# aapo-kossi/gym-eldorado

Measured on AMD Instinct MI355X. Metric: env-steps/sec at n_envs=65536, 4 players; bit-exact vs C++ ref, higher is better.
Workload: dtype u8; 1 GPU; C5: 65,536 envs in total over the ranks, 4 players, HARD, n_pieces=3, max_steps=100000, on-device masked sampler over selected_action_masks + step, persistent rollout kernel, every step's AoS outputs stored in HBM; n_envs_total=65536, n_envs_per_gpu=65536, seed=12345, parallelism=env-sharded x1 by index (runner.h:33-38 block split), no collectives

## Files before the change

gym-eldorado_amd/build_ext.py:

```python
from __future__ import annotations

import os
import subprocess
import sys
import sysconfig

PKG = os.path.dirname(os.path.abspath(__file__))
ROOT = os.path.dirname(PKG)
CSRC = os.path.join(PKG, "csrc")
OUT = os.path.join(PKG, "city_of_gold")
INCLUDE = os.path.join(ROOT, "include")
HIPCC = os.environ.get("HIPCC", "/opt/rocm/bin/hipcc")
ARCH = os.environ.get("COG_OFFLOAD_ARCH", "gfx950")

LIB = os.path.join(OUT, "libcog_hip.so")
LIB_FENCE = os.path.join(OUT, "libcog_hip_fence.so")
EXT = os.path.join(OUT, "_city_of_gold" + sysconfig.get_config_var("EXT_SUFFIX"))

ENGINE_SRCS = [os.path.join(CSRC, f) for f in ("cog_engine.hip", "cog_abi.cpp", "cog_policy.hip")]
ENGINE_DEPS = ENGINE_SRCS + [os.path.join(CSRC, f) for f in ("cog_engine.h", "cog_policy.h", "cog_tables.h", "cog_rng.h")] + [
    os.path.join(INCLUDE, f) for f in ("cog.h", "cog_types.h")]
EXT_SRCS = [os.path.join(CSRC, "pybind_module.cpp")]


def _stale(target, deps):
    if not os.path.exists(target):
        return True
    t = os.path.getmtime(target)
    return any(os.path.getmtime(d) > t for d in deps)


def _run(cmd, cwd=None):
    print("+", " ".join(cmd), flush=True)
    subprocess.run(cmd, check=True, cwd=cwd)


OBJ = os.path.join(PKG, "build")
HEADERS = [os.path.join(CSRC, f) for f in ("cog_engine.h", "cog_policy.h", "cog_tables.h", "cog_rng.h")] + [
    os.path.join(INCLUDE, f) for f in ("cog.h", "cog_types.h")]


def _compile_cmd(src, obj, defs=()):
    return [HIPCC, f"--offload-arch={ARCH}", "-O3", "-std=c++17", "-fPIC", "-c",
            "-ffp-contract=off", "-mllvm", "-amdgpu-sched-strategy=max-ilp", "-falign-loops=64", "-Wall",
            *defs, f"-I{INCLUDE}", f"-I{CSRC}", src, "-o", obj]


def build_engine(force=False, fence=True):
    os.makedirs(OBJ, exist_ok=True)
    jobs, objs = [], []
    for src in ENGINE_SRCS:
        obj = os.path.join(OBJ, os.path.basename(src) + ".o")
        objs.append(obj)
# ... 50 lines not shown
```

gym-eldorado_amd/csrc/cog_abi.cpp:

```cpp
#include <hip/hip_runtime.h>

#include <algorithm>
#include <atomic>
#include <chrono>
#include <cstdlib>
#include <cstring>
#include <mutex>
#include <random>
#include <string>
#include <vector>

#include "../../include/cog.h"
#include "cog_engine.h"
#include "cog_policy.h"

namespace {

thread_local std::string g_err;

int fail(int code, const std::string &msg) {
  g_err = msg;
  return code;
}

// ... 197 lines not shown
  size_t first = 0, n = 0;
  hipStream_t stream = nullptr;
  hipEvent_t ev = nullptr;
  cog::DevState s{};
  uint8_t *outs = nullptr;
  uint8_t *h_outs = nullptr;
  uint8_t *d_actions = nullptr;
  bool status_dirty = false;
  bool zc = false;
  uint8_t *h_obs_d = nullptr, *h_outs_d = nullptr, *mir = nullptr;
  bool mir_valid = false;
  bool host_synced = false, pub_done = false;
  Signal done;
  uint32_t park_seq = 0;
  uint64_t lean_clock = ~0ull;
  bool cdeck_ok = false;
};

struct cog_env {
  size_t n = 0;
  uint8_t n_players = 4;
  uint32_t max_steps = 0;
  uint64_t version = 0;
  std::vector<EnvShard> sh;
  uint32_t *h_err = nullptr;
  bool host = false;
  cog_obs_t *h_obs = nullptr;
  cog_action_mask_t *h_sel = nullptr;
  float *h_rew = nullptr;
  uint8_t *h_done = nullptr;
  uint8_t *h_agent = nullptr;
// ... 91 lines not shown

void env_free(cog_env *e) {
  if (!e) return;
  host_env_register(e, false);
  {
    std::lock_guard<std::mutex> lk(g_host_envs_mu);
    for (cog_sampler *q : g_samplers)
      if (q->spec.env == e) {
        q->spec.ok = false;
        q->spec.env = nullptr;
      }
  }
  for (EnvShard &k : e->sh) {
    DeviceGuard g(k.device);
    if (k.stream) (void)hipStreamSynchronize(k.stream);
    void *dev[] = {k.s.obs, k.outs, k.s.priv, k.s.grid, k.s.cgrid, k.s.heads, k.s.cdeck, k.s.cwide, k.s.gen, k.s.dirty, k.d_actions, k.mir,
                   k.s.park, k.s.parkq, k.done.ctr};
    for (void *p : dev)
      if (p) (void)hipFree(p);
    zc_free(k.h_outs);
    if (k.ev) (void)hipEventDestroy(k.ev);
    if (k.stream) (void)hipStreamDestroy(k.stream);
  }
  zc_free(e->h_obs);
  if (e->h_err) (void)hipHostFree(e->h_err);
  if (!single(e)) {
    void *more[] = {e->h_sel, e->h_rew, e->h_done, e->h_agent, e->h_info};
    for (void *p : more) zc_free(p);
  }
  delete e;
}
// ... 167 lines not shown
    DeviceGuard g(k.device);
    HIPCHK(hipMemcpyAsync(e->h_obs + k.first, k.s.obs, k.n * COG_OBS_BYTES, hipMemcpyDeviceToHost, k.stream));
    HIPCHK(hipMemcpyAsync(k.h_outs + kStatusBytes, k.outs + kStatusBytes, OutLayout(k.n).total - kStatusBytes,
                          hipMemcpyDeviceToHost, k.stream));
  }
  int rc = sync_all(e);
  if (rc) return rc;
  for (EnvShard &k : e->sh) k.mir_valid = false;
  gather_small(e);
  return COG_OK;
}

cog::DevState launch_state(const EnvShard &k, bool host_views) {
  cog::DevState s = k.s;
  if (!host_views) s.cap = 0;
  s.cdeck_ok = k.cdeck_ok ? 1u : 0u;
  return s;
}

void sampler_free(cog_sampler *s) {
  if (!s) return;
  sampler_register(s, false);
  if (!s->sh.empty()) {
    DeviceGuard g(s->sh[0].device);
    if (s->spec.d_rng) (void)hipFree(s->spec.d_rng);
    if (s->spec.d_actions) (void)hipFree(s->spec.d_actions);
  }
  zc_free(s->spec.h);
  for (SamplerShard &k : s->sh) {
    DeviceGuard g(k.device);
    if (k.stream) (void)hipStreamSynchronize(k.stream);
// ... 20 lines not shown
int env_shard_init(EnvShard &k, uint32_t default_seed, uint32_t *err_word) {
  DeviceGuard g(k.device);
  HIPCHK(hipStreamCreateWithFlags(&k.stream, hipStreamNonBlocking));
  HIPCHK(hipEventCreateWithFlags(&k.ev, hipEventDisableTiming));
  const size_t n = k.n;
  const OutLayout L(n);
  cog::DevState &s = k.s;
  int rc;
  if ((rc = dmalloc(&s.obs, n * COG_OBS_BYTES)) || (rc = dmalloc(&k.outs, L.alloc)) ||
      (rc = dmalloc(&s.priv, n * sizeof(cog::EnvPriv))) || (rc = dmalloc(&s.grid, n * (size_t)cog::kGridBytes)) ||
      (rc = dmalloc(&s.cgrid, n * (size_t)COG_CELLS)) || (rc = dmalloc(&s.heads, n * 5 * sizeof(uint4))) ||
      (rc = dmalloc(&s.gen, n * sizeof(cog::GenScratch))) || (rc = dmalloc(&s.dirty, n * sizeof(uint32_t))) ||
      (rc = dmalloc(&k.d_actions, n * COG_ACTION_BYTES)) || (rc = dmalloc(&s.park, n * sizeof(uint32_t))) ||
      (rc = dmalloc(&s.parkq, cog::park_list_bytes(n))) ||
      (rc = dmalloc(&k.done.ctr, 256)) || (rc = zc_alloc(&k.h_outs, L.alloc)) ||
      (rc = dmalloc(&s.cdeck, n * 10 * sizeof(uint4))) || (rc = dmalloc(&s.cwide, n * sizeof(uint32_t))))
    return rc;
  std::memset(k.h_outs, 0, L.alloc);
  s.n = n;
  s.first = k.first;
  s.cap = n;
  s.autoreset = 1;
  s.status = reinterpret_cast<uint32_t *>(k.outs);
  s.sel = k.outs + L.sel;
  s.info = k.outs + L.info;
  s.rew = reinterpret_cast<float *>(k.outs + L.rew);
  s.done = k.outs + L.done;
  s.agent = k.outs + L.agent;
  void *d_err = nullptr;
  HIPCHK(hipHostGetDevicePointer(&d_err, err_word, 0));
  s.err = static_cast<uint32_t *>(d_err);
// ... 95 lines not shown
  return COG_OK;
}

static int env_reset_impl(cog_env *e, const cog::ResetParams &p) {
  int rc = prepare_host(e);
  if (rc) return rc;
  env_changed(e);
  if (p.use_params) {
    e->n_players = p.n_players;
    e->max_steps = p.max_steps;
  }
  for (EnvShard &k : e->sh) {
    k.done.queued = false;
    k.host_synced = false;
    k.lean_clock = e->n_players >= 3 && e->max_steps ? 0ull : ~0ull;
    k.cdeck_ok = false;
  }
  for (EnvShard &k : e->sh) {
    DeviceGuard g(k.device);
    if (cog::launch_reset(k.s, p, k.stream) || cog::launch_encode_all(k.s, k.stream))
      return fail(COG_ERR_HIP, std::string("reset launch failed: ") + hipGetErrorString(hipGetLastError()));
    if ((rc = enqueue_status_only(k))) return rc;
  }
  if ((rc = sync_fast(e))) return rc;
  uint32_t flags = 0, errors = 0;
  for (size_t j = 0; j < e->sh.size(); j++) {
    EnvShard &k = e->sh[j];
    const uint32_t *st = reinterpret_cast<const uint32_t *>(k.h_outs);
    flags |= st[0];
    errors += st[1];
    if (st[0] || st[1] || st[2] || e->h_err[64 * j]) {
// ... 25 lines not shown

int cog_env_step_device_stream(cog_env *env, const void *d_actions, size_t n, void *stream) {
  if (!env || !d_actions) return fail(COG_ERR_INVALID, "NULL argument");
  if (n != env->n) return fail(COG_ERR_INVALID, "actions length != num_envs");
  if (!single(env)) return fail(COG_ERR_INVALID, "device actions need a single-shard env (one device pointer)");
  EnvShard &k = env->sh[0];
  DeviceGuard g(k.device);
  int rc = prepare_host(env);
  if (rc) return rc;
  env_changed(env);
  if (stream != COG_NO_STREAM) {
    HIPCHK(hipEventRecord(k.ev, static_cast<hipStream_t>(stream)));
    HIPCHK(hipStreamWaitEvent(k.stream, k.ev, 0));
  }
  k.lean_clock = ~0ull;
  k.cdeck_ok = false;
  if (cog::launch_step(launch_state(k, env->host), static_cast<const uint8_t *>(d_actions), k.stream))
    return fail(COG_ERR_HIP, std::string("step launch failed: ") + hipGetErrorString(hipGetLastError()));
  return finish(env, true);
}

int cog_env_step_device(cog_env *env, const void *d_actions, size_t n) {
  return cog_env_step_device_stream(env, d_actions, n, COG_NO_STREAM);
}

static bool spec_ready(cog_sampler *q) {
  SamplerSpec &sp = q->spec;
  if (sp.h) return true;
  DeviceGuard g(q->sh[0].device);
  if (dmalloc(&sp.d_rng, q->n * sizeof(uint32_t)) || dmalloc(&sp.d_actions, q->n * COG_ACTION_BYTES) ||
      zc_alloc(&sp.h, q->n * 8 + 64)) {
// ... 14 lines not shown
  if (q && (q->exported || q->sh[0].device != env->sh[0].device || std::getenv("COG_NO_SPEC") || !spec_ready(q)))
    q = nullptr;
  if (q) q->spec.ok = false;
  bool spec_launched = false;
  for (EnvShard &k : env->sh) {
    if (!k.n) continue;
    DeviceGuard g(k.device);
    const uint8_t *da = zc_device(actions + k.first, k.n * COG_ACTION_BYTES);
    if (!da || !zc_same_on(k.device, actions + k.first)) {
      HIPCHK(hipMemcpyAsync(k.d_actions, actions + k.first, k.n * COG_ACTION_BYTES, hipMemcpyHostToDevice, k.stream));
      da = k.d_actions;
    }
    uint32_t seq = 0, *ctr = nullptr;
    k.pub_done = false;
    k.lean_clock = ~0ull;
    k.cdeck_ok = false;
    if (env->host && k.zc && k.mir_valid && k.host_synced && cog::step_pub_ok(k.n) &&
        (ctr = signal_arm(k.done, seq))) {
      cog::DevState ps = launch_state(k, true);
      ps.pub_obs = k.h_obs_d;
      ps.pub_outs = k.h_outs_d;
      ps.pub_mir = k.mir;
      cog::SampleSpec sp{nullptr, nullptr, nullptr, nullptr, nullptr};
      if (q) {
        uint8_t *h = const_cast<uint8_t *>(zc_device(q->spec.h, n * 8 + 64));
        if (h) {
          *reinterpret_cast<volatile uint32_t *>(q->spec.h + n * 8) = 0u;
          sp = cog::SampleSpec{q->sh[0].d_rng, q->spec.d_rng, q->spec.d_actions, h, reinterpret_cast<uint32_t *>(h + n * 8)};
          spec_launched = true;
        }
      }
// ... 118 lines not shown
  }
  int rc = sync_all(env);
  if (rc) return rc;
  uint32_t acc = 0;
  for (uint32_t f : tmp) acc |= f;
  if (flags_or) *flags_or = acc;
  if (per_env) std::memcpy(per_env, tmp.data(), tmp.size() * sizeof(uint32_t));
  return COG_OK;
}

int cog_env_clear_hazards(cog_env *env) {
  if (!env) return fail(COG_ERR_INVALID, "env is NULL");
  for (EnvShard &k : env->sh) {
    if (!k.n) continue;
    DeviceGuard g(k.device);
    HIPCHK(hipMemset2DAsync(reinterpret_cast<uint8_t *>(k.s.priv) + offsetof(cog::EnvPriv, flags), sizeof(cog::EnvPriv),
                            0, sizeof(uint32_t), k.n, k.stream));
  }
  return sync_all(env);
}

int cog_env_time_encode(cog_env *env, int iters, int variant, double *ms_per_launch) {
  if (!env || iters < 1 || !ms_per_launch) return fail(COG_ERR_INVALID, "bad argument");
  EnvShard &k = env->sh[0];
  DeviceGuard g(k.device);
  hipEvent_t e0, e1;
  HIPCHK(hipEventCreate(&e0));
  HIPCHK(hipEventCreate(&e1));
  if (cog::launch_encode_all(k.s, k.stream, variant))
    return fail(COG_ERR_HIP, "encode launch failed");
// ... 86 lines not shown
  return COG_OK;
}

int cog_env_invalidate_device(cog_env *env, void *stream) {
  if (!env) return fail(COG_ERR_INVALID, "env is NULL");
  int rc = prepare_host(env);
  if (rc) return rc;
  env_changed(env);
  for (EnvShard &k : env->sh) {
    DeviceGuard g(k.device);
    if (stream != COG_NO_STREAM) {
      HIPCHK(hipEventRecord(k.ev, static_cast<hipStream_t>(stream)));
      HIPCHK(hipStreamWaitEvent(k.stream, k.ev, 0));
    }
    k.lean_clock = ~0ull;
    k.cdeck_ok = false;
    if (cog::launch_resync(k.s, k.stream))
      return fail(COG_ERR_HIP, std::string("resync launch failed: ") + hipGetErrorString(hipGetLastError()));
  }
  return finish(env, true);
}

int cog_env_set_autoreset(cog_env *env, int on) {
  if (!env) return fail(COG_ERR_INVALID, "env is NULL");
  int rc = sync_all(env);
  if (rc) return rc;
  env_changed(env);
  for (EnvShard &k : env->sh) {
    k.s.autoreset = on ? 1u : 0u;
    k.lean_clock = ~0ull;
    k.cdeck_ok = false;
  }
  return COG_OK;
}

int cog_sampler_create_multi(size_t n_envs, uint64_t seed, const int *devices, int n_devices, cog_sampler **out) {
  return cog_sampler_create_at(n_envs, seed, 0, devices, n_devices, out);
}

int cog_sampler_create_at(size_t n_envs, uint64_t seed, uint64_t first_index, const int *devices, int n_devices,
                          cog_sampler **out) {
  if (!out) return fail(COG_ERR_INVALID, "out is NULL");
  *out = nullptr;
  int rc = check_devices(devices, n_devices);
  if (rc) return rc;
  cog_sampler *s = new cog_sampler();
// ... 343 lines not shown
}

static int runner_launch_fused(cog_runner *r, int steps) {
  const int src = (r->flags & COG_RUNNER_STORED_MASKS) ? cog::MASK_STORED : cog::MASK_SELECTED;
  env_changed(r->env);
  r->smp->version++;
  const bool host = runner_host(r);
  int rc;
  if (host && (rc = prepare_host(r->env))) return rc;
  for (size_t j = 0; j < r->env->sh.size(); j++) {
    EnvShard &k = r->env->sh[j];
    SamplerShard &q = r->smp->sh[j];
    DeviceGuard g(k.device);
    if (host && steps == 1 && !r->timing && k.zc && k.mir_valid && k.host_synced && cog::step_pub_ok(k.n) && q.n) {
      k.lean_clock = ~0ull;
      k.cdeck_ok = false;
      uint8_t *h_act = const_cast<uint8_t *>(zc_device(r->smp->h_actions + q.first, q.n * COG_ACTION_BYTES));
      uint32_t seq = 0, *ctr = nullptr;
      if (h_act && zc_same_on(k.device, r->smp->h_actions + q.first) && (ctr = signal_arm(k.done, seq))) {
        cog::DevState ps = launch_state(k, true);
        ps.pub_obs = k.h_obs_d;
        ps.pub_outs = k.h_outs_d;
        ps.pub_mir = k.mir;
        if (cog::launch_sample_step_pub(ps, src, q.d_rng, q.d_actions, h_act, k.stream, ctr, k.done.d, seq))
          return fail(COG_ERR_HIP, std::string("sample_step launch failed: ") + hipGetErrorString(hipGetLastError()));
        signal_armed(k.done);
        k.pub_done = true;
        continue;
      }
    }
    views_pending(k);
    if (r->timing) {
      if ((rc = runner_timing_event(r, j))) return rc;
      HIPCHK(hipEventRecord(r->ev[j][r->ev_used], k.stream));
    }
    const cog::DevState s = launch_state(k, host);
    if (r->chunk > 1) {
      const bool trio = cog::rollout_kind_of(k.n, src, r->env->n_players >= 3) == 3;
      for (int t = 0; t < steps; t += r->chunk) {
        const int kk = std::min(r->chunk, steps - t);
        const bool no_fixup = trio && k.s.autoreset && k.lean_clock != ~0ull &&
                              k.lean_clock + (uint64_t)kk < (uint64_t)r->env->max_steps;
        cog::DevState sc = s;
        sc.cdeck_ok = trio && k.cdeck_ok ? 1u : 0u;
#ifdef COG_NO_CDECK
        sc.cdeck_ok = 0u;
#endif
        if (cog::launch_rollout(sc, src, kk, q.d_rng, q.d_actions, k.stream, r->env->n_players >= 3, &k.park_seq,
                                no_fixup))
          return fail(COG_ERR_HIP, std::string("rollout launch failed: ") + hipGetErrorString(hipGetLastError()));
        k.lean_clock = trio && k.lean_clock != ~0ull ? k.lean_clock + (uint64_t)kk : ~0ull;
        k.cdeck_ok = trio;
      }
    } else {
      k.lean_clock = ~0ull;
      k.cdeck_ok = false;
      for (int t = 0; t < steps; t++)
        if (cog::launch_sample_step(s, src, q.d_rng, q.d_actions, k.stream))
          return fail(COG_ERR_HIP, std::string("sample_step launch failed: ") + hipGetErrorString(hipGetLastError()));
    }
    if (r->timing) HIPCHK(hipEventRecord(r->ev[j][r->ev_used + 1], k.stream));
  }
  if (r->timing) {
    r->ev_used += 2;
    r->timed_launches += (uint64_t)steps;
  }
  return COG_OK;
}

int cog_runner_sample(cog_runner *r) {
  if (!r) return fail(COG_ERR_INVALID, "runner is NULL");
// ... 6 lines not shown
int cog_runner_step(cog_runner *r) {
  if (!r) return fail(COG_ERR_INVALID, "runner is NULL");
  env_changed(r->env);
  if (r->pending_sample) {
    r->pending_sample = false;
    return runner_launch_fused(r, 1);
  }
  const bool host = runner_host(r);
  int rc;
  if (host && (rc = prepare_host(r->env))) return rc;
  for (EnvShard &k : r->env->sh) views_pending(k);
  for (size_t j = 0; j < r->env->sh.size(); j++) {
    EnvShard &k = r->env->sh[j];
    DeviceGuard g(k.device);
    k.lean_clock = ~0ull;
    k.cdeck_ok = false;
    if (cog::launch_step(launch_state(k, host), r->smp->sh[j].d_actions, k.stream))
      return fail(COG_ERR_HIP, std::string("step launch failed: ") + hipGetErrorString(hipGetLastError()));
  }
  return COG_OK;
}

int cog_runner_rollout(cog_runner *r, int steps) {
  if (!r || steps < 0) return fail(COG_ERR_INVALID, "bad argument");
  int rc = runner_flush_sample(r);
  if (rc) return rc;
  return steps ? runner_launch_fused(r, steps) : COG_OK;
}

int cog_runner_sync(cog_runner *r) {
  if (!r) return fail(COG_ERR_INVALID, "runner is NULL");
// ... 53 lines not shown
```

gym-eldorado_amd/csrc/cog_engine.h:

```cpp
#pragma once
#include <stddef.h>
#include <stdint.h>

#include "../../include/cog_types.h"

namespace cog {

constexpr int kGridDim = 128;
constexpr int kGridOff = 64;
constexpr int kGridBytes = kGridDim * kGridDim;
#define COG_CELLS 2304
constexpr int kMaxCoord = 62;
constexpr int kMaxPlaced = 96;

constexpr uint32_t F_MAPGEN_FAIL = 0x01u;
constexpr uint32_t F_ERASE_PAST = 0x02u;
constexpr uint32_t F_Q9_OOB = 0x04u;
constexpr uint32_t F_Q24_CLAMP = 0x08u;
constexpr uint32_t F_GRID_OVER = 0x10u;
constexpr uint32_t F_OOB_LOOKUP = 0x20u;
constexpr uint32_t F_SCAN_OVER = 0x40u;
constexpr uint32_t F_B_START_LT4 = 0x80u;
constexpr uint32_t F_BAD_ACTION = 0x100u;
constexpr uint32_t F_SYNC_TIMEOUT = 0x200u;
// ... 34 lines not shown
};
static_assert(sizeof(GenScratch) <= 256, "GenScratch");

struct DevState {
  size_t n;
  uint8_t *obs;
  uint8_t *sel;
  uint8_t *info;
  float *rew;
  uint8_t *done;
  uint8_t *agent;
  EnvPriv *priv;
  uint8_t *grid;
  uint8_t *cgrid;
  uint4 *heads;
  uint4 *cdeck;
  uint32_t *cwide;
  GenScratch *gen;
  uint32_t *status;
  uint32_t *dirty;
  uint32_t *err;
  size_t first;
  size_t cap;
  uint32_t autoreset;
  unsigned long long *stamps;
  uint32_t *park;
  uint32_t *parkq;
  uint32_t park_par;
  uint32_t no_fixup;
  uint32_t trio_jt;
  uint32_t cdeck_ok;
  uint8_t *pub_obs, *pub_outs, *pub_mir;
  int32_t redo_at;
  int32_t redo_env;
};

struct ResetParams {
  uint32_t seed;
  uint8_t n_players, n_pieces, difficulty, use_params;
  uint32_t max_steps;
};

enum MaskSource : int { MASK_SELECTED = 0, MASK_STORED = 1, MASK_EXTERNAL = 2 };

int launch_init(const DevState &s, const uint32_t *seeds_host_unused, uint32_t default_seed,
                void *stream);
// ... 37 lines not shown
```

gym-eldorado_amd/csrc/cog_engine.hip:

```cpp
#include <hip/hip_runtime.h>
#include <algorithm>
#include <cstdlib>
#include <cstring>

#include "cog_engine.h"
#include "cog_tables.h"
#include "cog_rng.h"

#define DEV __device__ __forceinline__

#ifdef COG_STAMPS
DEV unsigned long long stamp_clock() {
  unsigned long long t;
  __builtin_amdgcn_sched_barrier(0);
  asm volatile("s_memtime %0\n\ts_waitcnt lgkmcnt(0)" : "=s"(t) :: "memory");
  __builtin_amdgcn_sched_barrier(0);
  return t;
}
#define STAMP(s, k)                                                                          \
  do {                                                                                       \
    const unsigned long long t_ = stamp_clock();                                             \
    if ((s).stamps && (threadIdx.x & 63) == 0)                                               \
      (s).stamps[((size_t)blockIdx.x * (blockDim.x / 64) + threadIdx.x / 64) * 16 + (k)] = t_; \
  } while (0)
// ... 2006 lines not shown

DEV void load_env(const DevState &s, size_t i, Snap &S) {
  const uint4 *pv4 = reinterpret_cast<const uint4 *>(s.priv + i);
  const uint4 *sh4 = reinterpret_cast<const uint4 *>(s.obs + i * COG_OBS_BYTES + COG_OBS_PHASE);
  S.g0 = pv4[0];
  S.g1 = pv4[1];
  S.g2 = pv4[2];
  S.info_steps = reinterpret_cast<const uint32_t *>(pv4 + 3)[0];
  S.sel = mbits_of(s.heads[5 * i]);
  S.sh[0] = sh4[0];
  S.sh[1] = sh4[1];
  S.sh[2] = sh4[2];
  const uint32_t w[5] = {S.sh[1].x, S.sh[1].y, S.sh[1].z, S.sh[1].w, S.sh[2].x};
  S.avail = shop_avail_of(w, (S.g1.y >> 8) & 0xffu, S.g1.z);
}
DEV uint8_t *deck_ptr(const DevState &s, size_t i, int p) {
  return s.obs + i * COG_OBS_BYTES + COG_OBS_PLAYER0 + COG_OBS_PLAYER_STRIDE * p;
}
DEV void load_players(const DevState &s, size_t i, int ag, int na, Snap &S) {
  const uint4 *pv4 = reinterpret_cast<const uint4 *>(s.priv + i);
  S.pla = pv4[4 + ag];
  S.pln = pv4[4 + na];
  S.ca = reinterpret_cast<const uint2 *>(pv4 + 8)[ag];
  S.cn = reinterpret_cast<const uint2 *>(pv4 + 8)[na];
  S.sta = mbits_of(s.heads[5 * i + 1 + ag]);
  S.stn = mbits_of(s.heads[5 * i + 1 + na]);
  const uint4 *dk = reinterpret_cast<const uint4 *>(deck_ptr(s, i, ag));
#pragma unroll
  for (int k = 0; k < 7; k++) S.dk[k] = dk[k];
}
// ... 382 lines not shown

constexpr uint32_t kParkNone = ~0u, kParkFinish = 1u << 31, kParkRedo = 1u << 30;
constexpr uint32_t kParkStep = kParkRedo - 1u;
DEV DevState wave_view(const DevState &s, size_t base) {
  DevState v = s;
  v.obs += base * COG_OBS_BYTES;
  v.sel += base * COG_MASK_BYTES;
  v.info += base * COG_INFO_BYTES;
  v.rew += base * 4;
  v.done += base;
  v.agent += base;
  v.priv += base;
  v.grid += base * (size_t)kGridBytes;
  v.cgrid += base * COG_CELLS;
  v.heads += 5 * base;
  v.cdeck += 10 * base;
  v.cwide += base;
  v.gen += base;
  v.park += base;
  v.first += base;
  v.n = s.n > base ? s.n - base : 0;
  return v;
}
DEV void park_list_push(const DevState &s_glob, bool parked) {
  if (__builtin_amdgcn_ballot_w64(parked) && (threadIdx.x & 63) == 0) {
    if (s_glob.no_fixup) {
      atomicOr(&s_glob.status[0], F_PARK_NOFIX);
      atomicAdd(&s_glob.status[1], 1u);
      *s_glob.err = 1u;
    }
    const uint32_t j = atomicAdd(&s_glob.parkq[s_glob.park_par], 1u);
// ... 787 lines not shown
  const int ne = (int)min((size_t)epw, s_glob.n - wbase);
  uint32_t *__restrict__ rngs = rngs_glob + wbase;
  bool live = l < ne;
  uint32_t park = kParkNone, srng = 0;
  PH_DECL;
  TL(10);
  RegEnv R;
  uint2 cells[4];
  int te1 = -1, te2 = -1;
  int ag = 0, na = 0;
  MBits selb = {0u, 0u, 0u}, stab = selb, stnb = selb;
  constexpr bool lat = LAT;
  uint4 pp = make_uint4(0u, 0u, 0u, 0u);
  uint32_t n_in_hand = 0u, n_active = 0u, steps_taken = 0u;
  uint32_t own = 0u;
  if (live) {
    Snap S;
    load_env(s, i, S);
    regs_env(R, S);
    const uint4 *pv4 = reinterpret_cast<const uint4 *>(s.priv + i);
#pragma unroll
    for (int p = 0; p < 4; p++) {
      D.pl[p][l] = pv4[4 + p];
      cells[p] = reinterpret_cast<const uint2 *>(pv4 + 8)[p];
      D.heads[p][l] = s.heads[5 * i + 1 + p];
    }
    srng = rngs[i];
    ag = (int)R.agent();
    na = (int)next_player((uint32_t)ag, R.n_players());
    pp = D.pl[ag][l];
    n_in_hand = (pp.y >> 8) & 0xffu;
    n_active = (pp.y >> 16) & 0xffu;
    steps_taken = (pp.z >> 8) & 0xffu;
#pragma unroll
    for (int p = 0; p < 4; p++) own |= (cells[p].x & 0xffu) << (8 * p);
    selb = S.sel;
    stab = mbits_of(D.heads[ag][l]);
    stnb = mbits_of(D.heads[na][l]);
  }
  R.tab = D.tab;
  __builtin_amdgcn_s_waitcnt(0);
// ... 177 lines not shown
      live = false;
    }
    ag = ag1;
    na = na1;
    PH(3);
  }
  TL(12);
  if (live && !lat) D.pl[ag][l] = pack_lean_player(pp, n_in_hand, n_active, steps_taken);
  cnt_store(D, CNT_REC, (uint32_t)steps + 1u);
  uint4 *pw = reinterpret_cast<uint4 *>(s.priv + i);
  if (lat) {
    if (live) {
      reinterpret_cast<uint3 *>(reinterpret_cast<uint32_t *>(pw) + 1)[0] = make_uint3(R.seed, R.max_steps, R.turn_counter);
      s.heads[5 * i] = mbits_u4(selb);
      rngs[i] = srng;
    }
    if (l < ne) s.park[i] = park;
    park_list_push(s_glob, park != kParkNone);
  }
  cnt_wait(D, cc, cc.fin, 3u, s_glob);
  PH(7);
  TL(13);
  const uint32_t fl = D.flg[l];
  if (lat) {
    if (live) pw[1] = make_uint4(R.g1x, R.g1y, R.in_market, R.flags | fl);
    else if (l < ne && fl) reinterpret_cast<uint32_t *>(pw)[7] = R.flags | fl;
  } else {
    if (live) {
      R.flags |= fl;
      trio_store_private(s, i, R, selb);
      rngs[i] = srng;
    } else if (l < ne && fl) {
      reinterpret_cast<uint32_t *>(pw)[7] = R.flags | fl;
    }
    if (l < ne) s.park[i] = park;
    park_list_push(s_glob, park != kParkNone);
  }
  trio_store_players(D, s, ne);
  PH(8);
  TL(14);
  PH_FLUSH(s_glob);
}

template <bool LAT>
DEV void trio_draw_play(TrioLds &D, const DevState &s, int l, bool live, int slot, uint32_t mt, uint32_t w2,
                        uint32_t gx, uint4 &p4, uint2 &h, uint2 &a, uint4 &shb0, uint32_t &infob, bool &te,
                        bool &rec_out, uint32_t &dm, uint32_t &nact) {
  const size_t i = (size_t)l;
  const int ag = (int)((mt >> 2) & 3u);
  const bool valid = live && (mt & kMetaValid);
  const bool rec = valid && (mt & kMetaStepped);
  rec_out = rec;
  te = rec && (int)(mt >> 24) != ag;
// ... 57 lines not shown

template <bool LAT>
DEV uint32_t trio_drawer(TrioLds &D, const DevState &s_glob, int steps, int epw) {
  PH_DECL;
  TL(14);
  const int l = (int)(threadIdx.x & 63);
  const size_t wbase = (size_t)blockIdx.x * epw;
  const DevState s = wave_view(s_glob, wbase);
  const size_t i = (size_t)l;
  const bool live = l < epw && wbase + (size_t)l < s_glob.n;
  uint32_t rng = 0u;
  bool narrow = true;
  constexpr bool lat = LAT;
  uint4 shb0 = make_uint4(0u, 0u, 0u, 0u);
  uint32_t infob = 0u;
  if (live && !s_glob.cdeck_ok) {
#pragma unroll
    for (int p = 0; p < 4; p++) {
      const uint4 *src = reinterpret_cast<const uint4 *>(deck_ptr(s, i, p));
      uint4 dk[7];
      uint2 pile[5];
#pragma unroll
      for (int k = 0; k < 7; k++) dk[k] = src[k];
      narrow = compact_of(dk, pile) && narrow;
#pragma unroll
      for (int q = 0; q < 5; q++) D.img[p][q][l] = pile[q];
    }
  }
  if (live) {
    rng = reinterpret_cast<const uint32_t *>(s.priv + i)[0];
    infob = reinterpret_cast<const uint32_t *>(s.priv + i)[12];
    shb0 = reinterpret_cast<const uint4 *>(s.obs + i * COG_OBS_BYTES + COG_OBS_PHASE)[0];
  }
  if (!s_glob.cdeck_ok) D.wide[l] = narrow ? 0u : 1u;
  uint32_t flags = 0u;
  __builtin_amdgcn_s_waitcnt(0);
  TL(15);
  __syncthreads();
  PH_RESET;
  TrioCnt6 cc;
  for (int r = 0; r < steps; r += 2) {
    const int nrec = r + 1 < steps ? 2 : 1;
    cnt_wait(D, cc, cc.rec, (uint32_t)(r + nrec), s_glob);
    PH(8);
    if (r + nrec >= steps) TL(11);
    const int slot[2] = {r & (kTrioDepth - 1), (r + 1) & (kTrioDepth - 1)};
    uint32_t dm[2] = {0u, 0u}, nact[2] = {0u, 0u};
    int agj[2] = {0, 0};
    bool te[2] = {false, false}, recj[2] = {false, false};
// ... 45 lines not shown
    }
#pragma unroll
    for (int j = 0; j < 2; j++)
      if (j < nrec) {
        uint32_t *w = &D.ring[slot[j]][2][l].w;
        if (lat && recj[j]) *w = (*w & 0xffu) | nact[j] << 8 | dm[j] << 16;
        else reinterpret_cast<uint16_t *>(w)[1] = (uint16_t)dm[j];
      }
    cnt_store(D, CNT_DRAW, (uint32_t)(r + nrec));
    PH(9);
  }
  TL(12);
  if (live) {
    reinterpret_cast<uint32_t *>(s.priv + i)[0] = rng;
    reinterpret_cast<uint32_t *>(s.priv + i)[12] = infob;
  }
  PH_FLUSH(s_glob);
  return flags;
}

template <int PART, bool LAT>
DEV uint32_t trio_storer(TrioLds &D, const DevState &s_glob, int steps, int epw, const uint32_t *__restrict__ rngs_glob,
                         uint8_t *__restrict__ actions_glob) {
  PH_DECL;
  TL(14);
  const int l = (int)(threadIdx.x & 63);
  const size_t wbase = (size_t)blockIdx.x * epw;
  const DevState s = wave_view(s_glob, wbase);
  const size_t i = (size_t)l;
  const bool live = l < epw && wbase + (size_t)l < s_glob.n;
  uint8_t *__restrict__ av = actions_glob + wbase * COG_ACTION_BYTES;
  MBits selb = {0u, 0u, 0u};
  uint2 cells[4];
  uint32_t out = ~0u;
  RegEnv E;
  E.flags = 0u;
  E.avail = 0u;
  uint32_t x = 1u;
  if (live) {
    if (PART == 0) {
      const uint4 *sh4 = reinterpret_cast<const uint4 *>(s.obs + i * COG_OBS_BYTES + COG_OBS_PHASE);
      const uint4 sh1 = sh4[1], sh2 = sh4[2];
      const uint4 *pv4 = reinterpret_cast<const uint4 *>(s.priv + i);
#pragma unroll
      for (int p = 0; p < 4; p++) {
        D.stbA[p][l] = s.heads[5 * i + 1 + p];
        cells[p] = reinterpret_cast<const uint2 *>(pv4 + 8)[p];
      }
      const uint4 g1 = pv4[1];
      const uint32_t w[5] = {sh1.x, sh1.y, sh1.z, sh1.w, sh2.x};
      E.avail = shop_avail_of(w, (g1.y >> 8) & 0xffu, g1.z);
      if (s_glob.cdeck_ok) {
        const uint4 *src = s.cdeck + 10 * i;
        uint4 c[10];
#pragma unroll
        for (int g = 0; g < 10; g++) c[g] = src[g];
#pragma unroll
        for (int g = 0; g < 10; g++) {
          D.img[(2 * g) / 5][(2 * g) % 5][l] = make_uint2(c[g].x, c[g].y);
          D.img[(2 * g + 1) / 5][(2 * g + 1) % 5][l] = make_uint2(c[g].z, c[g].w);
        }
      }
    } else {
      selb = mbits_of(s.heads[5 * i]);
      x = rngs_glob[wbase + (size_t)l];
    }
  }
  if (PART == 0 && s_glob.cdeck_ok) D.wide[l] = live ? s.cwide[i] : 0u;
  if (PART == 1) {
#pragma unroll
    for (int k = 0; k < kTrioLead; k++) {
      const uint4 p = presample(x);
      D.pre[k][l] = pre_pack(p, LAT);
      x = p.z;
    }
  }
  __builtin_amdgcn_s_waitcnt(0);
  TL(15);
  __syncthreads();
  PH_RESET;
  constexpr int LAG = PART == 1 ? kTrioBLag : 0;
  auto deck_rec = [&](int q) {
    const int sl = q & (kTrioDepth - 1);
// ... 74 lines not shown
        D.stbA[na][l] = mbits_u4(bn);
      }
    }
    if (PART == 1) {
      deck_rec(q);
    } else {
      cnt_store(D, CNT_STA, (uint32_t)(q + 1));
    }
    PH(13);
  }
  TL(12);
  if (PART == 0) {
    cnt_wait(D, cc, cc.rec, (uint32_t)steps + 1u, s_glob);
    if (live) {
#pragma unroll
      for (int p = 0; p < 4; p++) D.heads[p][l] = D.stbA[p][l];
      uint4 *dst = s.cdeck + 10 * i;
#pragma unroll
      for (int g = 0; g < 10; g++) {
        const uint2 a = D.img[(2 * g) / 5][(2 * g) % 5][l], b = D.img[(2 * g + 1) / 5][(2 * g + 1) % 5][l];
        dst[g] = make_uint4(a.x, a.y, b.x, b.y);
      }
      s.cwide[i] = D.wide[l];
    }
  }
  PH_FLUSH(s_glob);
  return E.flags;
}

template <int SRC, bool LAT>
__global__ void __launch_bounds__(256) __attribute__((amdgpu_waves_per_eu(4))) k_env_rollout_trio(DevState s, int steps, int epw, uint32_t *__restrict__ rngs,
                                                          uint8_t *__restrict__ actions_out) {
  __shared__ TrioLds D;
  const int role = __builtin_amdgcn_readfirstlane((int)(threadIdx.x >> 6));
  if (threadIdx.x < 64) D.flg[threadIdx.x] = 0u;
  if (threadIdx.x < kTrioCnts) D.cnt[threadIdx.x] = 0u;
// ... 13 lines not shown
  if (l == 0) __hip_atomic_fetch_add(&D.cnt[CNT_FIN], 1u, __ATOMIC_RELEASE, __HIP_MEMORY_SCOPE_WORKGROUP);
}

template <int SRC>
__global__ void __launch_bounds__(64) k_env_fixup(DevState s, int steps, uint32_t *__restrict__ rngs,
                                                  uint8_t *__restrict__ actions_out, int epw) {
  __shared__ LaneLds<64> L;
  const uint32_t cnt = s.parkq[s.park_par];
  if (blockIdx.x >= cnt) return;
  uid_tab_fill(L.tab);
  for (uint32_t w = blockIdx.x; w < cnt; w += gridDim.x) {
    const size_t base = (size_t)s.parkq[2 + w] * (size_t)epw;
    const size_t i0 = base + threadIdx.x;
    const uint32_t park = (int)threadIdx.x < epw && i0 < s.n ? s.park[i0] : kParkNone;
    rollout_pass<SRC, true, 64>(L, s, steps, rngs, actions_out, park, nullptr, base);
    if (park != kParkNone) {
      const int l = (int)threadIdx.x;
      uint4 *pw = reinterpret_cast<uint4 *>(s.priv + i0);
#pragma unroll
      for (int p = 0; p < 4; p++) {
        pw[4 + p] = L.pl[p][l];
        reinterpret_cast<uint2 *>(pw + 8)[p] = L.cells[p][l];
        s.heads[5 * i0 + 1 + p] = L.heads[p][l];
      }
      bool narrow = true;
#pragma unroll
      for (int p = 0; p < 4; p++) {
        const uint4 *src = reinterpret_cast<const uint4 *>(deck_ptr(s, i0, p));
        uint4 dk[7];
        uint2 pile[5];
#pragma unroll
        for (int k = 0; k < 7; k++) dk[k] = src[k];
        narrow = compact_of(dk, pile) && narrow;
        uint2 *dst = reinterpret_cast<uint2 *>(s.cdeck + 10 * i0) + 5 * p;
#pragma unroll
        for (int q = 0; q < 5; q++) dst[q] = pile[q];
      }
      s.cwide[i0] = narrow ? 0u : 1u;
      s.park[i0] = kParkNone;
    }
  }
}

__global__ void __launch_bounds__(256) k_sample(size_t n, const uint8_t *__restrict__ masks,
                                                uint32_t *__restrict__ rngs, uint8_t *__restrict__ actions,
                                                uint8_t *__restrict__ h_actions, GridSignal sig) {
  __shared__ UidEntry tab[kUidTab];
  uid_tab_fill(tab);
  const size_t i = (size_t)blockIdx.x * blockDim.x + threadIdx.x;
  if (i < n) {
    uint32_t rng = rngs[i];
    uint8_t a[5];
// ... 305 lines not shown
    }();
    DevState sd = s;
    sd.redo_at = park_nofix.first >= 0 ? park_nofix.first : redo_at;
    sd.redo_env = park_nofix.first >= 0 ? (int32_t)park_nofix.second : -1;
    sd.park_par = (*park_seq)++ & 1u;
    static const bool always_fixup = getenv("COG_ALWAYS_FIXUP") != nullptr;
    sd.no_fixup = no_fixup && kind == RK_TRIO && (redo_at < 0 || park_nofix.first >= 0) && !always_fixup ? 1u : 0u;
    const int epw = kind == RK_TRIO ? trio_epw(s.n) : 64;
    const unsigned nb = blocks_for(s.n, epw);
    const dim3 g(nb), gf(fixup_grid(nb));
    static const int jt_env = [] {
      const char *e = getenv("COG_TRIO_JT");
      return e && *e ? atoi(e) : -1;
    }();
    sd.trio_jt = jt_env >= 0 ? (uint32_t)(jt_env != 0) : (nb <= cu_shape().cus ? 1u : 0u);
    if (mask_source == MASK_STORED) {
      hipLaunchKernelGGL((k_env_rollout_duo<MASK_STORED>), g, dim3(128), 0, st, sd, steps, d_rng, d_actions);
      hipLaunchKernelGGL((k_env_fixup<MASK_STORED>), gf, dim3(64), 0, st, sd, steps, d_rng, d_actions, epw);
    } else if (kind == RK_TRIO) {
      if (sd.trio_jt)
        hipLaunchKernelGGL((k_env_rollout_trio<MASK_SELECTED, true>), g, dim3(256), trio_pad_lds(nb), st, sd, steps, epw,
                           d_rng, d_actions);
      else
        hipLaunchKernelGGL((k_env_rollout_trio<MASK_SELECTED, false>), g, dim3(256), trio_pad_lds(nb), st, sd, steps, epw,
                           d_rng, d_actions);
      if (!sd.no_fixup)
        hipLaunchKernelGGL((k_env_fixup<MASK_SELECTED>), gf, dim3(64), 0, st, sd, steps, d_rng, d_actions, epw);
    } else {
      hipLaunchKernelGGL((k_env_rollout_duo<MASK_SELECTED>), g, dim3(128), 0, st, sd, steps, d_rng, d_actions);
      hipLaunchKernelGGL((k_env_fixup<MASK_SELECTED>), gf, dim3(64), 0, st, sd, steps, d_rng, d_actions, epw);
// ... 77 lines not shown
```

Measured before the change: 25.89 billion env-steps/s.

## Carry per-env rollout state across launches in a coalesced SoA carry buffer

Replaces the per-env compact deck buffer with a wider carry buffer laid out in 64-env blocks of 28 uint4 planes, so each lane reads and writes one 16-byte granule per plane. The buffer holds decks, private globals, player state, cells, heads and shop words. Later rollout launches reload state from it with coalesced loads instead of scattered AoS reads from priv, heads and obs. The cost is extra stores on every launch to keep the carry current, plus invalidation logic at reset and on every non-trio path; a stale carry would break bit-exactness.

```diff
diff --git a/gym-eldorado_amd/build_ext.py b/gym-eldorado_amd/build_ext.py
--- a/gym-eldorado_amd/build_ext.py
+++ b/gym-eldorado_amd/build_ext.py
@@ -18,7 +18,7 @@
 EXT = os.path.join(OUT, "_city_of_gold" + sysconfig.get_config_var("EXT_SUFFIX"))
 
 ENGINE_SRCS = [os.path.join(CSRC, f) for f in ("cog_engine.hip", "cog_abi.cpp", "cog_policy.hip")]
-ENGINE_DEPS = ENGINE_SRCS + [os.path.join(CSRC, f) for f in ("cog_engine.h", "cog_policy.h", "cog_tables.h", "cog_rng.h")] + [
+ENGINE_DEPS = ENGINE_SRCS + [os.path.join(CSRC, f) for f in ("cog_engine.h", "cog_policy.h", "cog_tables.h", "cog_rng.h", "cog_carry.h")] + [
     os.path.join(INCLUDE, f) for f in ("cog.h", "cog_types.h")]
 EXT_SRCS = [os.path.join(CSRC, "pybind_module.cpp")]
 
@@ -36,7 +36,7 @@
 
 
 OBJ = os.path.join(PKG, "build")
-HEADERS = [os.path.join(CSRC, f) for f in ("cog_engine.h", "cog_policy.h", "cog_tables.h", "cog_rng.h")] + [
+HEADERS = [os.path.join(CSRC, f) for f in ("cog_engine.h", "cog_policy.h", "cog_tables.h", "cog_rng.h", "cog_carry.h")] + [
     os.path.join(INCLUDE, f) for f in ("cog.h", "cog_types.h")]
 
 
diff --git a/gym-eldorado_amd/csrc/cog_abi.cpp b/gym-eldorado_amd/csrc/cog_abi.cpp
--- a/gym-eldorado_amd/csrc/cog_abi.cpp
+++ b/gym-eldorado_amd/csrc/cog_abi.cpp
@@ -235,7 +235,7 @@
   Signal done;
   uint32_t park_seq = 0;
   uint64_t lean_clock = ~0ull;
-  bool cdeck_ok = false;
+  bool carry_ok = false;
 };
 
 struct cog_env {
@@ -357,7 +357,7 @@
   for (EnvShard &k : e->sh) {
     DeviceGuard g(k.device);
     if (k.stream) (void)hipStreamSynchronize(k.stream);
-    void *dev[] = {k.s.obs, k.outs, k.s.priv, k.s.grid, k.s.cgrid, k.s.heads, k.s.cdeck, k.s.cwide, k.s.gen, k.s.dirty, k.d_actions, k.mir,
+    void *dev[] = {k.s.obs, k.outs, k.s.priv, k.s.grid, k.s.cgrid, k.s.heads, k.s.carry, k.s.cwide, k.s.gen, k.s.dirty, k.d_actions, k.mir,
                    k.s.park, k.s.parkq, k.done.ctr};
     for (void *p : dev)
       if (p) (void)hipFree(p);
@@ -555,7 +555,7 @@
 cog::DevState launch_state(const EnvShard &k, bool host_views) {
   cog::DevState s = k.s;
   if (!host_views) s.cap = 0;
-  s.cdeck_ok = k.cdeck_ok ? 1u : 0u;
+  s.carry_ok = k.carry_ok ? 1u : 0u;
   return s;
 }
 
@@ -606,7 +606,7 @@
       (rc = dmalloc(&k.d_actions, n * COG_ACTION_BYTES)) || (rc = dmalloc(&s.park, n * sizeof(uint32_t))) ||
       (rc = dmalloc(&s.parkq, cog::park_list_bytes(n))) ||
       (rc = dmalloc(&k.done.ctr, 256)) || (rc = zc_alloc(&k.h_outs, L.alloc)) ||
-      (rc = dmalloc(&s.cdeck, n * 10 * sizeof(uint4))) || (rc = dmalloc(&s.cwide, n * sizeof(uint32_t))))
+      (rc = dmalloc(&s.carry, cog::carry_granules(n) * sizeof(uint4))) || (rc = dmalloc(&s.cwide, n * sizeof(uint32_t))))
     return rc;
   std::memset(k.h_outs, 0, L.alloc);
   s.n = n;
@@ -732,7 +732,7 @@
     k.done.queued = false;
     k.host_synced = false;
     k.lean_clock = e->n_players >= 3 && e->max_steps ? 0ull : ~0ull;
-    k.cdeck_ok = false;
+    k.carry_ok = false;
   }
   for (EnvShard &k : e->sh) {
     DeviceGuard g(k.device);
@@ -788,7 +788,7 @@
     HIPCHK(hipStreamWaitEvent(k.stream, k.ev, 0));
   }
   k.lean_clock = ~0ull;
-  k.cdeck_ok = false;
+  k.carry_ok = false;
   if (cog::launch_step(launch_state(k, env->host), static_cast<const uint8_t *>(d_actions), k.stream))
     return fail(COG_ERR_HIP, std::string("step launch failed: ") + hipGetErrorString(hipGetLastError()));
   return finish(env, true);
@@ -833,7 +833,7 @@
     uint32_t seq = 0, *ctr = nullptr;
     k.pub_done = false;
     k.lean_clock = ~0ull;
-    k.cdeck_ok = false;
+    k.carry_ok = false;
     if (env->host && k.zc && k.mir_valid && k.host_synced && cog::step_pub_ok(k.n) &&
         (ctr = signal_arm(k.done, seq))) {
       cog::DevState ps = launch_state(k, true);
@@ -982,6 +982,7 @@
   for (EnvShard &k : env->sh) {
     if (!k.n) continue;
     DeviceGuard g(k.device);
+    k.carry_ok = false;
     HIPCHK(hipMemset2DAsync(reinterpret_cast<uint8_t *>(k.s.priv) + offsetof(cog::EnvPriv, flags), sizeof(cog::EnvPriv),
                             0, sizeof(uint32_t), k.n, k.stream));
   }
@@ -1098,7 +1099,7 @@
       HIPCHK(hipStreamWaitEvent(k.stream, k.ev, 0));
     }
     k.lean_clock = ~0ull;
-    k.cdeck_ok = false;
+    k.carry_ok = false;
     if (cog::launch_resync(k.s, k.stream))
       return fail(COG_ERR_HIP, std::string("resync launch failed: ") + hipGetErrorString(hipGetLastError()));
   }
@@ -1113,7 +1114,7 @@
   for (EnvShard &k : env->sh) {
     k.s.autoreset = on ? 1u : 0u;
     k.lean_clock = ~0ull;
-    k.cdeck_ok = false;
+    k.carry_ok = false;
   }
   return COG_OK;
 }
@@ -1487,7 +1488,7 @@
     DeviceGuard g(k.device);
     if (host && steps == 1 && !r->timing && k.zc && k.mir_valid && k.host_synced && cog::step_pub_ok(k.n) && q.n) {
       k.lean_clock = ~0ull;
-      k.cdeck_ok = false;
+      k.carry_ok = false;
       uint8_t *h_act = const_cast<uint8_t *>(zc_device(r->smp->h_actions + q.first, q.n * COG_ACTION_BYTES));
       uint32_t seq = 0, *ctr = nullptr;
       if (h_act && zc_same_on(k.device, r->smp->h_actions + q.first) && (ctr = signal_arm(k.done, seq))) {
@@ -1515,19 +1516,19 @@
         const bool no_fixup = trio && k.s.autoreset && k.lean_clock != ~0ull &&
                               k.lean_clock + (uint64_t)kk < (uint64_t)r->env->max_steps;
         cog::DevState sc = s;
-        sc.cdeck_ok = trio && k.cdeck_ok ? 1u : 0u;
+        sc.carry_ok = trio && k.carry_ok ? 1u : 0u;
 #ifdef COG_NO_CDECK
-        sc.cdeck_ok = 0u;
+        sc.carry_ok = 0u;
 #endif
         if (cog::launch_rollout(sc, src, kk, q.d_rng, q.d_actions, k.stream, r->env->n_players >= 3, &k.park_seq,
                                 no_fixup))
           return fail(COG_ERR_HIP, std::string("rollout launch failed: ") + hipGetErrorString(hipGetLastError()));
         k.lean_clock = trio && k.lean_clock != ~0ull ? k.lean_clock + (uint64_t)kk : ~0ull;
-        k.cdeck_ok = trio;
+        k.carry_ok = trio;
       }
     } else {
       k.lean_clock = ~0ull;
-      k.cdeck_ok = false;
+      k.carry_ok = false;
       for (int t = 0; t < steps; t++)
         if (cog::launch_sample_step(s, src, q.d_rng, q.d_actions, k.stream))
           return fail(COG_ERR_HIP, std::string("sample_step launch failed: ") + hipGetErrorString(hipGetLastError()));
@@ -1564,7 +1565,7 @@
     EnvShard &k = r->env->sh[j];
     DeviceGuard g(k.device);
     k.lean_clock = ~0ull;
-    k.cdeck_ok = false;
+    k.carry_ok = false;
     if (cog::launch_step(launch_state(k, host), r->smp->sh[j].d_actions, k.stream))
       return fail(COG_ERR_HIP, std::string("step launch failed: ") + hipGetErrorString(hipGetLastError()));
   }
diff --git a/gym-eldorado_amd/csrc/cog_carry.h b/gym-eldorado_amd/csrc/cog_carry.h
--- /dev/null
+++ b/gym-eldorado_amd/csrc/cog_carry.h
@@ -0,0 +1,29 @@
+#pragma once
+#include <stddef.h>
+#include <stdint.h>
+
+#ifndef COG_HD
+#define COG_HD __host__ __device__ __forceinline__
+#endif
+
+namespace cog {
+
+enum CarryPlane : int {
+  kCarryDeck = 0,
+  kCarryG0 = 10,
+  kCarryG1 = 11,
+  kCarryG2 = 12,
+  kCarryDraw = 13,
+  kCarryPl = 14,
+  kCarryCells = 18,
+  kCarryHeads = 20,
+  kCarryObs = 25,
+  kCarryPlanes = 28
+};
+constexpr size_t kCarryBlock = 64;
+
+COG_HD size_t carry_granules(size_t n) { return (n + kCarryBlock - 1) / kCarryBlock * (size_t)kCarryPlanes * kCarryBlock; }
+COG_HD size_t carry_base(size_t e) { return e / kCarryBlock * (size_t)kCarryPlanes * kCarryBlock + e % kCarryBlock; }
+COG_HD size_t carry_slot(size_t e, int g) { return carry_base(e) + (size_t)g * kCarryBlock; }
+
+}
diff --git a/gym-eldorado_amd/csrc/cog_engine.h b/gym-eldorado_amd/csrc/cog_engine.h
--- a/gym-eldorado_amd/csrc/cog_engine.h
+++ b/gym-eldorado_amd/csrc/cog_engine.h
@@ -3,6 +3,7 @@
 #include <stdint.h>
 
 #include "../../include/cog_types.h"
+#include "cog_carry.h"
 
 namespace cog {
 
@@ -72,7 +73,7 @@
   uint8_t *grid;
   uint8_t *cgrid;
   uint4 *heads;
-  uint4 *cdeck;
+  uint4 *carry;
   uint32_t *cwide;
   GenScratch *gen;
   uint32_t *status;
@@ -87,7 +88,7 @@
   uint32_t park_par;
   uint32_t no_fixup;
   uint32_t trio_jt;
-  uint32_t cdeck_ok;
+  uint32_t carry_ok;
   uint8_t *pub_obs, *pub_outs, *pub_mir;
   int32_t redo_at;
   int32_t redo_env;
diff --git a/gym-eldorado_amd/csrc/cog_engine.hip b/gym-eldorado_amd/csrc/cog_engine.hip
--- a/gym-eldorado_amd/csrc/cog_engine.hip
+++ b/gym-eldorado_amd/csrc/cog_engine.hip
@@ -2044,6 +2044,18 @@
   const uint32_t w[5] = {S.sh[1].x, S.sh[1].y, S.sh[1].z, S.sh[1].w, S.sh[2].x};
   S.avail = shop_avail_of(w, (S.g1.y >> 8) & 0xffu, S.g1.z);
 }
+DEV void load_env_carry(const uint4 *ci, Snap &S) {
+  S.g0 = ci[64 * kCarryG0];
+  S.g1 = ci[64 * kCarryG1];
+  S.g2 = ci[64 * kCarryG2];
+  S.info_steps = 0u;
+  S.sel = mbits_of(ci[64 * kCarryHeads]);
+  S.sh[0] = ci[64 * kCarryObs];
+  S.sh[1] = ci[64 * (kCarryObs + 1)];
+  S.sh[2] = ci[64 * (kCarryObs + 2)];
+  const uint32_t w[5] = {S.sh[1].x, S.sh[1].y, S.sh[1].z, S.sh[1].w, S.sh[2].x};
+  S.avail = shop_avail_of(w, (S.g1.y >> 8) & 0xffu, S.g1.z);
+}
 DEV uint8_t *deck_ptr(const DevState &s, size_t i, int p) {
   return s.obs + i * COG_OBS_BYTES + COG_OBS_PLAYER0 + COG_OBS_PLAYER_STRIDE * p;
 }
@@ -2456,7 +2468,7 @@
   v.grid += base * (size_t)kGridBytes;
   v.cgrid += base * COG_CELLS;
   v.heads += 5 * base;
-  v.cdeck += 10 * base;
+  v.carry += carry_base(base);
   v.cwide += base;
   v.gen += base;
   v.park += base;
@@ -3274,17 +3286,37 @@
   uint4 pp = make_uint4(0u, 0u, 0u, 0u);
   uint32_t n_in_hand = 0u, n_active = 0u, steps_taken = 0u;
   uint32_t own = 0u;
+  uint4 *const ci = s.carry + l;
   if (live) {
     Snap S;
-    load_env(s, i, S);
+    if (s_glob.carry_ok) {
+      load_env_carry(ci, S);
+      const uint4 c0 = ci[64 * kCarryCells], c1 = ci[64 * (kCarryCells + 1)];
+      cells[0] = make_uint2(c0.x, c0.y);
+      cells[1] = make_uint2(c0.z, c0.w);
+      cells[2] = make_uint2(c1.x, c1.y);
+      cells[3] = make_uint2(c1.z, c1.w);
+#pragma unroll
+      for (int p = 0; p < 4; p++) {
+        D.pl[p][l] = ci[64 * (kCarryPl + p)];
+        D.heads[p][l] = ci[64 * (kCarryHeads + 1 + p)];
+      }
+    } else {
+      load_env(s, i, S);
+      const uint4 *pv4 = reinterpret_cast<const uint4 *>(s.priv + i);
+#pragma unroll
+      for (int p = 0; p < 4; p++) {
+        D.pl[p][l] = pv4[4 + p];
+        cells[p] = reinterpret_cast<const uint2 *>(pv4 + 8)[p];
+        D.heads[p][l] = s.heads[5 * i + 1 + p];
+      }
+      ci[64 * kCarryG2] = S.g2;
+      ci[64 * kCarryCells] = make_uint4(cells[0].x, cells[0].y, cells[1].x, cells[1].y);
+      ci[64 * (kCarryCells + 1)] = make_uint4(cells[2].x, cells[2].y, cells[3].x, cells[3].y);
+      ci[64 * (kCarryObs + 1)] = S.sh[1];
+      ci[64 * (kCarryObs + 2)] = S.sh[2];
+    }
     regs_env(R, S);
-    const uint4 *pv4 = reinterpret_cast<const uint4 *>(s.priv + i);
-#pragma unroll
-    for (int p = 0; p < 4; p++) {
-      D.pl[p][l] = pv4[4 + p];
-      cells[p] = reinterpret_cast<const uint2 *>(pv4 + 8)[p];
-      D.heads[p][l] = s.heads[5 * i + 1 + p];
-    }
     srng = rngs[i];
     ag = (int)R.agent();
     na = (int)next_player((uint32_t)ag, R.n_players());
@@ -3492,6 +3524,8 @@
       reinterpret_cast<uint3 *>(reinterpret_cast<uint32_t *>(pw) + 1)[0] = make_uint3(R.seed, R.max_steps, R.turn_counter);
       s.heads[5 * i] = mbits_u4(selb);
       rngs[i] = srng;
+      ci[64 * kCarryG0] = make_uint4(0u, R.seed, R.max_steps, R.turn_counter);
+      ci[64 * kCarryHeads] = mbits_u4(selb);
     }
     if (l < ne) s.park[i] = park;
     park_list_push(s_glob, park != kParkNone);
@@ -3501,13 +3535,18 @@
   TL(13);
   const uint32_t fl = D.flg[l];
   if (lat) {
-    if (live) pw[1] = make_uint4(R.g1x, R.g1y, R.in_market, R.flags | fl);
-    else if (l < ne && fl) reinterpret_cast<uint32_t *>(pw)[7] = R.flags | fl;
+    if (live) {
+      pw[1] = make_uint4(R.g1x, R.g1y, R.in_market, R.flags | fl);
+      ci[64 * kCarryG1] = make_uint4(R.g1x, R.g1y, R.in_market, R.flags | fl);
+    } else if (l < ne && fl) reinterpret_cast<uint32_t *>(pw)[7] = R.flags | fl;
   } else {
     if (live) {
       R.flags |= fl;
       trio_store_private(s, i, R, selb);
       rngs[i] = srng;
+      ci[64 * kCarryG0] = make_uint4(0u, R.seed, R.max_steps, R.turn_counter);
+      ci[64 * kCarryG1] = make_uint4(R.g1x, R.g1y, R.in_market, R.flags);
+      ci[64 * kCarryHeads] = mbits_u4(selb);
     } else if (l < ne && fl) {
       reinterpret_cast<uint32_t *>(pw)[7] = R.flags | fl;
     }
@@ -3515,6 +3554,10 @@
     park_list_push(s_glob, park != kParkNone);
   }
   trio_store_players(D, s, ne);
+  if (l < ne) {
+#pragma unroll
+    for (int p = 0; p < 4; p++) ci[64 * (kCarryPl + p)] = D.pl[p][l];
+  }
   PH(8);
   TL(14);
   PH_FLUSH(s_glob);
@@ -3602,7 +3645,8 @@
   constexpr bool lat = LAT;
   uint4 shb0 = make_uint4(0u, 0u, 0u, 0u);
   uint32_t infob = 0u;
-  if (live && !s_glob.cdeck_ok) {
+  uint4 *const ci = s.carry + l;
+  if (live && !s_glob.carry_ok) {
 #pragma unroll
     for (int p = 0; p < 4; p++) {
       const uint4 *src = reinterpret_cast<const uint4 *>(deck_ptr(s, i, p));
@@ -3615,12 +3659,17 @@
       for (int q = 0; q < 5; q++) D.img[p][q][l] = pile[q];
     }
   }
-  if (live) {
+  if (live && s_glob.carry_ok) {
+    const uint4 dw = ci[64 * kCarryDraw];
+    infob = dw.x;
+    rng = dw.y;
+    shb0 = ci[64 * kCarryObs];
+  } else if (live) {
     rng = reinterpret_cast<const uint32_t *>(s.priv + i)[0];
     infob = reinterpret_cast<const uint32_t *>(s.priv + i)[12];
     shb0 = reinterpret_cast<const uint4 *>(s.obs + i * COG_OBS_BYTES + COG_OBS_PHASE)[0];
   }
-  if (!s_glob.cdeck_ok) D.wide[l] = narrow ? 0u : 1u;
+  if (!s_glob.carry_ok) D.wide[l] = narrow ? 0u : 1u;
   uint32_t flags = 0u;
   __builtin_amdgcn_s_waitcnt(0);
   TL(15);
@@ -3696,6 +3745,8 @@
   if (live) {
     reinterpret_cast<uint32_t *>(s.priv + i)[0] = rng;
     reinterpret_cast<uint32_t *>(s.priv + i)[12] = infob;
+    ci[64 * kCarryDraw] = make_uint4(infob, rng, 0u, 0u);
+    ci[64 * kCarryObs] = shb0;
   }
   PH_FLUSH(s_glob);
   return flags;
@@ -3719,24 +3770,39 @@
   E.flags = 0u;
   E.avail = 0u;
   uint32_t x = 1u;
+  uint4 *const ci = s.carry + l;
   if (live) {
     if (PART == 0) {
-      const uint4 *sh4 = reinterpret_cast<const uint4 *>(s.obs + i * COG_OBS_BYTES + COG_OBS_PHASE);
-      const uint4 sh1 = sh4[1], sh2 = sh4[2];
-      const uint4 *pv4 = reinterpret_cast<const uint4 *>(s.priv + i);
-#pragma unroll
-      for (int p = 0; p < 4; p++) {
-        D.stbA[p][l] = s.heads[5 * i + 1 + p];
-        cells[p] = reinterpret_cast<const uint2 *>(pv4 + 8)[p];
-      }
-      const uint4 g1 = pv4[1];
+      uint4 sh1, sh2, g1;
+      if (s_glob.carry_ok) {
+        sh1 = ci[64 * (kCarryObs + 1)];
+        sh2 = ci[64 * (kCarryObs + 2)];
+        g1 = ci[64 * kCarryG1];
+        const uint4 c0 = ci[64 * kCarryCells], c1 = ci[64 * (kCarryCells + 1)];
+        cells[0] = make_uint2(c0.x, c0.y);
+        cells[1] = make_uint2(c0.z, c0.w);
+        cells[2] = make_uint2(c1.x, c1.y);
+        cells[3] = make_uint2(c1.z, c1.w);
+#pragma unroll
+        for (int p = 0; p < 4; p++) D.stbA[p][l] = ci[64 * (kCarryHeads + 1 + p)];
+      } else {
+        const uint4 *sh4 = reinterpret_cast<const uint4 *>(s.obs + i * COG_OBS_BYTES + COG_OBS_PHASE);
+        sh1 = sh4[1];
+        sh2 = sh4[2];
+        const uint4 *pv4 = reinterpret_cast<const uint4 *>(s.priv + i);
+#pragma unroll
+        for (int p = 0; p < 4; p++) {
+          D.stbA[p][l] = s.heads[5 * i + 1 + p];
+          cells[p] = reinterpret_cast<const uint2 *>(pv4 + 8)[p];
+        }
+        g1 = pv4[1];
+      }
       const uint32_t w[5] = {sh1.x, sh1.y, sh1.z, sh1.w, sh2.x};
       E.avail = shop_avail_of(w, (g1.y >> 8) & 0xffu, g1.z);
-      if (s_glob.cdeck_ok) {
-        const uint4 *src = s.cdeck + 10 * i;
+      if (s_glob.carry_ok) {
         uint4 c[10];
 #pragma unroll
-        for (int g = 0; g < 10; g++) c[g] = src[g];
+        for (int g = 0; g < 10; g++) c[g] = ci[64 * (kCarryDeck + g)];
 #pragma unroll
         for (int g = 0; g < 10; g++) {
           D.img[(2 * g) / 5][(2 * g) % 5][l] = make_uint2(c[g].x, c[g].y);
@@ -3744,11 +3810,11 @@
         }
       }
     } else {
-      selb = mbits_of(s.heads[5 * i]);
+      selb = mbits_of(s_glob.carry_ok ? ci[64 * kCarryHeads] : s.heads[5 * i]);
       x = rngs_glob[wbase + (size_t)l];
     }
   }
-  if (PART == 0 && s_glob.cdeck_ok) D.wide[l] = live ? s.cwide[i] : 0u;
+  if (PART == 0 && s_glob.carry_ok) D.wide[l] = live ? s.cwide[i] : 0u;
   if (PART == 1) {
 #pragma unroll
     for (int k = 0; k < kTrioLead; k++) {
@@ -3853,12 +3919,15 @@
     cnt_wait(D, cc, cc.rec, (uint32_t)steps + 1u, s_glob);
     if (live) {
 #pragma unroll
-      for (int p = 0; p < 4; p++) D.heads[p][l] = D.stbA[p][l];
-      uint4 *dst = s.cdeck + 10 * i;
+      for (int p = 0; p < 4; p++) {
+        const uint4 h = D.stbA[p][l];
+        D.heads[p][l] = h;
+        ci[64 * (kCarryHeads + 1 + p)] = h;
+      }
 #pragma unroll
       for (int g = 0; g < 10; g++) {
         const uint2 a = D.img[(2 * g) / 5][(2 * g) % 5][l], b = D.img[(2 * g + 1) / 5][(2 * g + 1) % 5][l];
-        dst[g] = make_uint4(a.x, a.y, b.x, b.y);
+        ci[64 * (kCarryDeck + g)] = make_uint4(a.x, a.y, b.x, b.y);
       }
       s.cwide[i] = D.wide[l];
     }
@@ -3902,6 +3971,7 @@
     const size_t i0 = base + threadIdx.x;
     const uint32_t park = (int)threadIdx.x < epw && i0 < s.n ? s.park[i0] : kParkNone;
     rollout_pass<SRC, true, 64>(L, s, steps, rngs, actions_out, park, nullptr, base);
+    __builtin_amdgcn_fence(__ATOMIC_ACQ_REL, "workgroup");
     if (park != kParkNone) {
       const int l = (int)threadIdx.x;
       uint4 *pw = reinterpret_cast<uint4 *>(s.priv + i0);
@@ -3911,19 +3981,35 @@
         reinterpret_cast<uint2 *>(pw + 8)[p] = L.cells[p][l];
         s.heads[5 * i0 + 1 + p] = L.heads[p][l];
       }
+      uint4 *ci = s.carry + carry_base(i0);
       bool narrow = true;
+      uint2 cd[20];
 #pragma unroll
       for (int p = 0; p < 4; p++) {
         const uint4 *src = reinterpret_cast<const uint4 *>(deck_ptr(s, i0, p));
         uint4 dk[7];
-        uint2 pile[5];
 #pragma unroll
         for (int k = 0; k < 7; k++) dk[k] = src[k];
-        narrow = compact_of(dk, pile) && narrow;
-        uint2 *dst = reinterpret_cast<uint2 *>(s.cdeck + 10 * i0) + 5 * p;
-#pragma unroll
-        for (int q = 0; q < 5; q++) dst[q] = pile[q];
-      }
+        narrow = compact_of(dk, cd + 5 * p) && narrow;
+      }
+#pragma unroll
+      for (int g = 0; g < 10; g++) ci[64 * (kCarryDeck + g)] = make_uint4(cd[2 * g].x, cd[2 * g].y, cd[2 * g + 1].x, cd[2 * g + 1].y);
+      const uint4 g0 = pw[0], g3 = pw[3];
+      ci[64 * kCarryG0] = g0;
+      ci[64 * kCarryG1] = pw[1];
+      ci[64 * kCarryG2] = pw[2];
+      ci[64 * kCarryDraw] = make_uint4(g3.x, g0.x, 0u, 0u);
+      ci[64 * kCarryHeads] = s.heads[5 * i0];
+#pragma unroll
+      for (int p = 0; p < 4; p++) {
+        ci[64 * (kCarryPl + p)] = L.pl[p][l];
+        ci[64 * (kCarryHeads + 1 + p)] = L.heads[p][l];
+      }
+      ci[64 * kCarryCells] = make_uint4(L.cells[0][l].x, L.cells[0][l].y, L.cells[1][l].x, L.cells[1][l].y);
+      ci[64 * (kCarryCells + 1)] = make_uint4(L.cells[2][l].x, L.cells[2][l].y, L.cells[3][l].x, L.cells[3][l].y);
+      const uint4 *sh4 = reinterpret_cast<const uint4 *>(s.obs + i0 * COG_OBS_BYTES + COG_OBS_PHASE);
+#pragma unroll
+      for (int k = 0; k < 3; k++) ci[64 * (kCarryObs + k)] = sh4[k];
       s.cwide[i0] = narrow ? 0u : 1u;
       s.park[i0] = kParkNone;
     }
@@ -4259,6 +4345,11 @@
       return e && *e ? atoi(e) : -1;
     }();
     sd.trio_jt = jt_env >= 0 ? (uint32_t)(jt_env != 0) : (nb <= cu_shape().cus ? 1u : 0u);
+    static const bool carry_on = [] {
+      const char *e = getenv("COG_TRIO_CARRY");
+      return !(e && *e == '0');
+    }();
+    if (!carry_on) sd.carry_ok = 0u;
     if (mask_source == MASK_STORED) {
       hipLaunchKernelGGL((k_env_rollout_duo<MASK_STORED>), g, dim3(128), 0, st, sd, steps, d_rng, d_actions);
       hipLaunchKernelGGL((k_env_fixup<MASK_STORED>), gf, dim3(64), 0, st, sd, steps, d_rng, d_actions, epw);
```

Result: no change. 25.80 billion env-steps/s (-0.4%).
